# geoeo/ORB_SLAM3_V1.0

Hardware: AMD Instinct MI355X
Metric: frames/sec ORB extract+match, 752x480 8-level 1000-feat; bit-exact kp/desc (higher is better)
Workload: dtype u8

## Files before the change

### orb_slam3_v1.0_amd/csrc/kernels_pyramid.hip

```cpp
#include <algorithm>
#include <cstdlib>

#include "launch.h"

namespace orbfe {

constexpr int kRsTW = 128, kRsTH = 16;
constexpr int kRsMaxRows = 40, kRsMaxCols = 304;

template <int KPASS>
__global__ __launch_bounds__(256) void resize_kernel(const uint8_t* __restrict__ src, size_t srcFrameStride,
                                                     int sw, int sh, int spitch, int srcAligned4,
                                                     uint8_t* __restrict__ dst, size_t dstFrameStride,
                                                     int dw, int dh, int dpitch,
                                                     const uint32_t* __restrict__ xtab,
                                                     const uint32_t* __restrict__ ytab)
{
    __shared__ __attribute__((aligned(16))) uint8_t sSrc[kRsMaxRows][kRsMaxCols];

    const int f = blockIdx.x;
    const int tx0 = blockIdx.y * kRsTW;
    const int ty0 = blockIdx.z * kRsTH;
    const int tid = threadIdx.x;
    const uint8_t* s = src + (size_t)f * srcFrameStride;

    const int x0 = tx0 + (tid & 31) * 4;
    const int yA = ty0 + (tid >> 5), yB = yA + 8;
    const bool colOk = x0 < dw;
    uint4 xt4 = make_uint4(0, 0, 0, 0);
    uint32_t ytA = 0, ytB = 0;
    if (colOk) xt4 = *reinterpret_cast<const uint4*>(xtab + x0);
    if (yA < dh) ytA = ytab[yA];
    if (yB < dh) ytB = ytab[yB];

    const int txLast = min(tx0 + kRsTW, dw) - 1;
    const int tyLast = min(ty0 + kRsTH, dh) - 1;
    const int sx0 = (int)(xtab[tx0] & 0xffffu) & ~3;
    const int sx1 = min((int)(xtab[txLast] & 0xffffu) + 1, sw - 1);
    const int sy0 = (int)(ytab[ty0] & 0xffffu);
    const int sy1 = min((int)(ytab[tyLast] & 0xffffu) + 1, sh - 1);
    const int nrows = sy1 - sy0 + 1;
    const int ndw = (sx1 - sx0) / 4 + 1;
    const bool staged = nrows <= 4 * KPASS && ndw * 4 <= kRsMaxCols;

    if (staged) {
        const int c4l = tid & 63, rl = tid >> 6;
        if (srcAligned4 && ndw <= 64) {
            constexpr int kPass = KPASS;
            const bool cok = c4l < ndw;
            uint32_t off = __umul24((unsigned)(sy0 + rl), (unsigned)spitch) + (unsigned)(sx0 + 4 * c4l);
            const uint32_t step = 4u * (unsigned)spitch;
            uint32_t wv[kPass];
#pragma unroll
            for (int k = 0; k < kPass; k++) {
                wv[k] = 0;
                if (cok && rl + 4 * k < nrows) wv[k] = *reinterpret_cast<const uint32_t*>(s + off);
                off += step;
            }
#pragma unroll
            for (int k = 0; k < kPass; k++)
                if (cok && rl + 4 * k < nrows) *reinterpret_cast<uint32_t*>(&sSrc[rl + 4 * k][4 * c4l]) = wv[k];
        } else {
            for (int r = rl; r < nrows; r += 4) {
                const uint8_t* row = s + (size_t)(sy0 + r) * spitch;
                for (int c4 = c4l; c4 < ndw; c4 += 64) {
                    const int gx = sx0 + 4 * c4;
                    uint32_t wv = 0;
#pragma unroll
                    for (int i = 0; i < 4; i++)
                        if (gx + i < sw) wv |= (uint32_t)row[gx + i] << (8 * i);
                    *reinterpret_cast<uint32_t*>(&sSrc[r][4 * c4]) = wv;
                }
            }
        }
        __syncthreads();
    }
    if (!colOk) return;

    const uint32_t xt[4] = {xt4.x, xt4.y, xt4.z, xt4.w};
    const int nvalid = min(4, dw - x0);
    auto body = [&](auto fetch) {
#pragma unroll
        for (int half = 0; half < 2; half++) {
            const int y = half ? yB : yA;
            if (y >= dh) continue;
            const uint32_t yt = half ? ytB : ytA;
            const int y1 = (int)(yt & 0xffffu);
            const uint32_t wy = yt >> 16;
            const int y2 = min(y1 + 1, sh - 1);
            uint32_t outw = 0;
            const uint32_t wyc = 2048u - wy;
#pragma unroll
            for (int i = 0; i < 4; i++) {
                const int x1 = (int)(xt[i] & 0xffffu);
                const uint32_t wx = xt[i] >> 16;
                const uint32_t wxc = 2048u - wx;
                const int x2 = min(x1 + 1, sw - 1);
                const uint32_t a = fetch(y1, x1), b = fetch(y1, x2), c = fetch(y2, x1), e = fetch(y2, x2);
                const uint32_t top = __umul24(a, wxc) + __umul24(b, wx);
                const uint32_t bot = __umul24(c, wxc) + __umul24(e, wx);
                const uint32_t v = __umul24(top, wyc) + __umul24(bot, wy) + (1u << 21);
                outw |= (v >> 22) << (8 * i);
            }
            uint8_t* d = dst + (size_t)f * dstFrameStride + __umul24((unsigned)y, (unsigned)dpitch);
            if (nvalid == 4) {
                *reinterpret_cast<uint32_t*>(d + x0) = outw;
            } else {
                for (int i = 0; i < nvalid; i++) d[x0 + i] = (uint8_t)(outw >> (8 * i));
            }
        }
    };
    if (staged)
        body([&](int yy, int xx) -> uint32_t {
            return (&sSrc[0][0])[__umul24((uint32_t)(yy - sy0), (uint32_t)kRsMaxCols) + (uint32_t)(xx - sx0)];
        });
    else
        body([&](int yy, int xx) -> uint32_t { return s[(size_t)yy * spitch + xx]; });
}


constexpr int kPyrWaves = 4;

constexpr int kPyrRows = 7;
constexpr int kPyrSegDw = 96;
constexpr int kPyrStride = 128;


__device__ __forceinline__ uint32_t mad24_vsv(uint32_t a, uint32_t w, uint32_t c)
{
    uint32_t r;
    asm("v_mad_u32_u24 %0, %1, %2, %3" : "=v"(r) : "v"(a), "s"(w), "v"(c));
    return r;
}

__device__ __forceinline__ void pyr_hpass(uint32_t d0, uint32_t d1, uint32_t d2, const uint32_t (&sel)[4], const uint32_t (&wp)[4],
                                          uint32_t (&h)[4])
{
    typedef unsigned short us2 __attribute__((ext_vector_type(2)));
    const uint32_t e0 = __builtin_amdgcn_alignbyte(d1, d0, 3), e1 = __builtin_amdgcn_alignbyte(d2, d1, 3);
#pragma unroll
    for (int i = 0; i < 4; i++) {
        const uint32_t pair = i < 3 ? __builtin_amdgcn_perm(d1, d0, sel[i]) : __builtin_amdgcn_perm(e1, e0, sel[i]);
        h[i] = __builtin_amdgcn_udot2(__builtin_bit_cast(us2, pair), __builtin_bit_cast(us2, wp[i]), 0u, false);
    }
}

__global__ __launch_bounds__(kPyrWaves * 64) void pyramid_kernel(const PipelineDesc* __restrict__ P, int l, int R,
                                                                 const uint8_t* __restrict__ gray0, size_t gray0FrameStride,
                                                                 int gray0Pitch, uint8_t* __restrict__ ws,
                                                                 const uint32_t* __restrict__ tabs)
{
    __shared__ uint32_t sRows[kPyrWaves][kPyrRows][kPyrStride];

    const int f = blockIdx.x;
    const int lane = threadIdx.x & 63;
    const int wave = __builtin_amdgcn_readfirstlane((int)(threadIdx.x >> 6));
    uint32_t* const ring = &sRows[wave][0][0];

    {
        const LevelDesc& S = P->lv[l - 1];
        const LevelDesc& D = P->lv[l];
        const int sw = S.w, sh = S.h, dw = D.w, dh = D.h, dpitch = D.pitch;
        const uint8_t* src = l == 1 ? gray0 + (size_t)f * gray0FrameStride : ws + S.imgOff + (size_t)f * S.imgFrameStride;
        const int spitch = l == 1 ? gray0Pitch : S.pitch;
        uint8_t* dst = ws + D.imgOff + (size_t)f * D.imgFrameStride;
        const uint32_t* xtab = tabs + D.xtabOff;
        const uint32_t* ytab = tabs + D.ytabOff;
        const int strips = (dh + R - 1) / R, chunks = (dw + 255) / 256;
        const __amdgpu_buffer_rsrc_t srsrc =
            __builtin_amdgcn_make_buffer_rsrc(const_cast<uint8_t*>(src), 0, (sh - 1) * spitch + ((sw + 3) & ~3), 0x00020000);
        const __amdgpu_buffer_rsrc_t drsrc = __builtin_amdgcn_make_buffer_rsrc(dst, 0, dh * dpitch, 0x00020000);

        const int task = (int)blockIdx.y * kPyrWaves + wave;
        if (task < strips * chunks) {
            const int strip = task / chunks, chunk = task - strip * chunks;
            const int x0 = chunk * 256 + lane * 4;
            const bool colOk = x0 < dw;
            const int xg = min(x0, (dw - 1) & ~3);
            const uint4 xt4 = *reinterpret_cast<const uint4*>(xtab + xg);
            const uint32_t xt[4] = {xt4.x, xt4.y, xt4.z, xt4.w};
            const uint32_t start = (xt[0] & 0xffffu) & ~3u;
            const uint32_t segBase = (xtab[chunk * 256] & 0xffffu) & ~3u;
            const uint32_t winOff = start - segBase;
            uint32_t sel[4], wp[4];
#pragma unroll
            for (int i = 0; i < 4; i++) {
                const uint32_t o = (xt[i] & 0xffffu) - start - (i == 3 ? 3u : 0u);
                sel[i] = 0x0c000c00u | o | ((o + 1u) << 16);
                const uint32_t wx = xt[i] >> 16;
                wp[i] = (2048u - wx) | (wx << 16);
            }
            const int nvalid = min(4, dw - x0);
            constexpr uint32_t kNowhere = 0x7ffffff0u;
            const uint32_t rowEnd = (uint32_t)((sw + 3) & ~3);
            const uint32_t colA = segBase + 4u * (uint32_t)lane;
            const uint32_t ldA = colA + 4u <= rowEnd ? colA : kNowhere;
            const uint32_t ldB = (lane < kPyrSegDw - 64 && colA + 260u <= rowEnd) ? colA + 256u : kNowhere;
            const uint32_t stX = colOk ? (uint32_t)x0 : kNowhere;
            const bool partial = (dw & 3) != 0;

            const int ys = strip * R, ye = min(ys + R, dh);
            const uint32_t roMax = (uint32_t)((sh - 1) * spitch);
            uint32_t kRound = 1u << 23;
            asm("" : "+v"(kRound));
            uint32_t ytN[4];
            uint32_t ga[kPyrRows], gb[kPyrRows];
            auto request = [&](int yb) {
                const uint4 y4 = *reinterpret_cast<const uint4*>(ytab + yb);
                ytN[0] = y4.x; ytN[1] = y4.y; ytN[2] = y4.z; ytN[3] = y4.w;
                uint32_t ro = (ytN[0] & 0xffffu) * (uint32_t)spitch;
#pragma unroll
                for (int j = 0; j < kPyrRows; j++) {
                    const uint32_t roc = min(ro, roMax);
                    ga[j] = __builtin_amdgcn_raw_buffer_load_b32(srsrc, ldA, roc, 0);
                    gb[j] = __builtin_amdgcn_raw_buffer_load_b32(srsrc, ldB, roc, 0);
                    ro += (uint32_t)spitch;
                }
            };
            request(ys);
            uint32_t stRow = (uint32_t)(ys * dpitch);
#pragma unroll 1
            for (int yb = ys; yb < ye; yb += 4) {
                uint32_t yt[4];
#pragma unroll
                for (int k = 0; k < 4; k++) yt[k] = ytN[k];
                const int rA = (int)(yt[0] & 0xffffu);
#pragma unroll
                for (int j = 0; j < kPyrRows; j++) {
                    ring[j * kPyrStride + lane] = ga[j];
                    ring[j * kPyrStride + 64 + lane] = gb[j];
                }
                if (yb + 4 < ye) request(yb + 4);
#pragma unroll
                for (int k = 0; k < 4; k++) {
                    const int jt = (int)(yt[k] & 0xffffu) - rA;
                    const uint32_t* wt = reinterpret_cast<const uint32_t*>(reinterpret_cast<const uint8_t*>(ring + jt * kPyrStride) + winOff);
                    const uint32_t* wb = wt + kPyrStride;
                    uint32_t hT[4], hB[4];
                    pyr_hpass(wt[0], wt[1], wt[2], sel, wp, hT);
                    pyr_hpass(wb[0], wb[1], wb[2], sel, wp, hB);
                    const uint32_t wy4 = (yt[k] >> 16) * 4u, wyc4 = 8192u - wy4;
                    uint32_t v[4];
#pragma unroll
                    for (int i = 0; i < 4; i++) v[i] = mad24_vsv(hB[i], wy4, mad24_vsv(hT[i], wyc4, kRound));
                    const uint32_t lo = __builtin_amdgcn_perm(v[1], v[0], 0x0c0c0703u);
                    const uint32_t hi = __builtin_amdgcn_perm(v[3], v[2], 0x0c0c0703u);
                    const uint32_t outw = lo | (hi << 16);
                    if (yb + k < ye) {
                        if (!partial) {
                            __builtin_amdgcn_raw_buffer_store_b32(outw, drsrc, stX, stRow, 0);
                        } else if (colOk) {
                            if (nvalid == 4) {
                                __builtin_amdgcn_raw_buffer_store_b32(outw, drsrc, (uint32_t)x0, stRow, 0);
                            } else {
                                for (int i = 0; i < nvalid; i++)
                                    __builtin_amdgcn_raw_buffer_store_b8((uint8_t)(outw >> (8 * i)), drsrc, (uint32_t)(x0 + i), stRow, 0);
                            }
                        }
                    }
                    stRow += (uint32_t)dpitch;
                }
            }
        }
    }
}

void launch_resize(hipStream_t s, int frames, const uint8_t* src, size_t srcFrameStride, int sw, int sh,
                   int spitch, int srcAligned4, uint8_t* dst, size_t dstFrameStride, int dw, int dh, int dpitch,
                   const uint32_t* xtab, const uint32_t* ytab)
{
    dim3 block(256);
    dim3 grid(frames, (dw + kRsTW - 1) / kRsTW, (dh + kRsTH - 1) / kRsTH);
    const int maxRows = (int)(((long long)(kRsTH - 1) * sh + dh - 1) / dh) + 2;
    if (maxRows <= 24)
        hipLaunchKernelGGL(resize_kernel<6>, grid, block, 0, s, src, srcFrameStride, sw, sh, spitch, srcAligned4, dst,
                           dstFrameStride, dw, dh, dpitch, xtab, ytab);
    else
        hipLaunchKernelGGL(resize_kernel<kRsMaxRows / 4>, grid, block, 0, s, src, srcFrameStride, sw, sh, spitch, srcAligned4,
                           dst, dstFrameStride, dw, dh, dpitch, xtab, ytab);
}


bool pyramid_level_fits(const uint32_t* xtab, const uint32_t* ytab, int sw, int sh, int dw, int dh)
{
    for (int y = 0; y < dh; y++) {
        if ((int)(ytab[y] & 0xffffu) + 1 > sh - 1) return false;
        const int yl = std::min(y + 3, dh - 1);
        if ((int)(ytab[yl] & 0xffffu) + 1 - (int)(ytab[y] & 0xffffu) + 1 > kPyrRows) return false;
    }
    for (int c0 = 0; c0 < dw; c0 += 256) {
        const uint32_t segBase = (xtab[c0] & 0xffffu) & ~3u;
        const int xl = (std::min(c0 + 256, dw) - 1) & ~3;
        const uint32_t startL = (xtab[xl] & 0xffffu) & ~3u;
        if (startL + 12 - segBase > 4u * kPyrSegDw) return false;
    }
    for (int x0 = 0; x0 < dw; x0 += 4) {
        const uint32_t start = (xtab[x0] & 0xffffu) & ~3u;
        for (int i = 0; i < 4 && x0 + i < dw; i++) {
            const uint32_t x1 = xtab[x0 + i] & 0xffffu;
            if ((int)x1 + 1 > sw - 1 || x1 < start) return false;
            const uint32_t o = x1 - start;
            if (i < 3 ? o + 1 > 7 : (o < 3 || o - 3 + 1 > 7)) return false;
        }
    }
    return true;
}

void launch_pyramid_level(hipStream_t s, int frames, const PipelineDesc* dP, int level, int dw, int dh, const uint8_t* gray0,
                          size_t gray0FrameStride, int gray0Pitch, uint8_t* ws, const uint32_t* tabs)
{
#ifdef ORBFE_DIAG
    static const int envR = getenv("ORBFE_PYR_ROWS") ? atoi(getenv("ORBFE_PYR_ROWS")) : 0;
#else
    constexpr int envR = 0;
#endif
    const int R = envR > 0 ? (envR + 3) & ~3 : frames >= 128 ? 8 : 4;
    const int tasks = ((dh + R - 1) / R) * ((dw + 255) / 256);
    hipLaunchKernelGGL(pyramid_kernel, dim3(frames, (tasks + kPyrWaves - 1) / kPyrWaves), dim3(kPyrWaves * 64), 0, s, dP, level, R, gray0,
                       gray0FrameStride, gray0Pitch, ws, tabs);
}


namespace {

struct ChainCtx {
    const uint8_t* src0;
    int pitch0, w0, h0;
    const uint32_t* xtab[3];
    const uint32_t* ytab[3];
    int w[3], h[3];
};

template <int K>
__device__ __forceinline__ uint32_t chain_px(const ChainCtx& c, int x, int y)
{
    const uint32_t xt = c.xtab[K - 1][x], yt = c.ytab[K - 1][y];
    const int sw = K == 1 ? c.w0 : c.w[K - 2], sh = K == 1 ? c.h0 : c.h[K - 2];
    const int x1 = (int)(xt & 0xffffu), y1 = (int)(yt & 0xffffu);
    const uint32_t wx = xt >> 16, wy = yt >> 16;
    const uint32_t wxc = 2048u - wx, wyc = 2048u - wy;
    const int x2 = min(x1 + 1, sw - 1), y2 = min(y1 + 1, sh - 1);
    uint32_t a, b, cc, e;
    if constexpr (K == 1) {
        const uint8_t* r1 = c.src0 + (size_t)y1 * c.pitch0;
        const uint8_t* r2 = c.src0 + (size_t)y2 * c.pitch0;
        a = r1[x1]; b = r1[x2]; cc = r2[x1]; e = r2[x2];
    } else {
        a = chain_px<K - 1>(c, x1, y1); b = chain_px<K - 1>(c, x2, y1);
        cc = chain_px<K - 1>(c, x1, y2); e = chain_px<K - 1>(c, x2, y2);
    }
    const uint32_t top = __umul24(a, wxc) + __umul24(b, wx);
    const uint32_t bot = __umul24(cc, wxc) + __umul24(e, wx);
    const uint32_t v = __umul24(top, wyc) + __umul24(bot, wy) + (1u << 21);
    return v >> 22;
}

__global__ __launch_bounds__(256) void pyramid_chain_kernel(const PipelineDesc* __restrict__ P, int l0, int depth,
                                                            const uint8_t* __restrict__ gray0, size_t gray0FrameStride, int gray0Pitch,
                                                            uint8_t* __restrict__ ws, const uint32_t* __restrict__ tabs,
                                                            uint32_t* __restrict__ zero, int nZeroPerFrame)
{
    const int f = blockIdx.y;
    if (zero && blockIdx.x == 0)
        for (int i = threadIdx.x; i < nZeroPerFrame; i += 256) zero[(size_t)f * nZeroPerFrame + i] = 0;
    ChainCtx c;
    const LevelDesc& S = P->lv[l0];
    c.src0 = l0 == 0 ? gray0 + (size_t)f * gray0FrameStride : ws + S.imgOff + (size_t)f * S.imgFrameStride;
    c.pitch0 = l0 == 0 ? gray0Pitch : S.pitch;
    c.w0 = S.w;
    c.h0 = S.h;
    int np[3] = {0, 0, 0};
#pragma unroll
    for (int k = 0; k < 3; k++) {
        const LevelDesc& D = P->lv[min(l0 + 1 + k, P->nLevels - 1)];
        c.xtab[k] = tabs + D.xtabOff;
        c.ytab[k] = tabs + D.ytabOff;
        c.w[k] = D.w;
        c.h[k] = D.h;
        np[k] = k < depth ? D.w * D.h : 0;
    }
    int idx = (int)blockIdx.x * 256 + (int)threadIdx.x;
    int k = 0;
    if (idx >= np[0]) { idx -= np[0]; k = 1; if (idx >= np[1]) { idx -= np[1]; k = 2; if (idx >= np[2]) return; } }
    const LevelDesc& D = P->lv[l0 + 1 + k];
    const int y = idx / D.w, x = idx - y * D.w;
    uint32_t out;
    if (k == 0) out = chain_px<1>(c, x, y);
    else if (k == 1) out = chain_px<2>(c, x, y);
    else out = chain_px<3>(c, x, y);
    ws[D.imgOff + (size_t)f * D.imgFrameStride + (size_t)y * D.pitch + x] = (uint8_t)out;
}

}

void launch_pyramid_chain(hipStream_t s, int frames, const PipelineDesc* dP, const PipelineDesc& hostP, int l0, int depth,
                          const uint8_t* gray0, size_t gray0FrameStride, int gray0Pitch, uint8_t* ws, const uint32_t* tabs,
                          uint32_t* zero, int nZeroPerFrame)
{
    long long pixels = 0;
    for (int k = 0; k < depth; k++) {
        const LevelDesc& D = hostP.lv[l0 + 1 + k];
        pixels += (long long)D.w * D.h;
    }
    hipLaunchKernelGGL(pyramid_chain_kernel, dim3((unsigned)((pixels + 255) / 256), frames), dim3(256), 0, s, dP, l0, depth, gray0,
                       gray0FrameStride, gray0Pitch, ws, tabs, zero, nZeroPerFrame);
}

}
```

Baseline: 226,900.

## Stream pyramid rows through a two-slot LDS ring and reuse horizontal passes across rows

The pyramid kernel stops staging all seven source rows per quad into a 7-row LDS ring. Each row is now written into a double-buffered two-row slot, horizontally filtered once, and the result is carried forward as hPrev. Output rows are emitted as soon as their bottom row's pass is ready, and a row already filtered by the previous quad is skipped via the carry check. It also prefetches the ytab quads ahead, interleaves the next quad's global loads with the per-row work, and simplifies tail stores. This cuts LDS footprint and duplicate horizontal filtering, but adds a stricter monotonic-ytab fit check and more complex control flow.

```diff
diff --git a/orb_slam3_v1.0_amd/csrc/kernels_pyramid.hip b/orb_slam3_v1.0_amd/csrc/kernels_pyramid.hip
--- a/orb_slam3_v1.0_amd/csrc/kernels_pyramid.hip
+++ b/orb_slam3_v1.0_amd/csrc/kernels_pyramid.hip
@@ -1,5 +1,6 @@
 #include <algorithm>
 #include <cstdlib>
+#include <type_traits>
 
 #include "launch.h"
 
@@ -123,7 +124,8 @@
 
 constexpr int kPyrRows = 7;
 constexpr int kPyrSegDw = 96;
-constexpr int kPyrStride = 128;
+constexpr int kPyrSlack = kPyrRows - 5;
+constexpr int kPyrMinLast = 4;
 
 
 __device__ __forceinline__ uint32_t mad24_vsv(uint32_t a, uint32_t w, uint32_t c)
@@ -150,7 +152,7 @@
                                                                  int gray0Pitch, uint8_t* __restrict__ ws,
                                                                  const uint32_t* __restrict__ tabs)
 {
-    __shared__ uint32_t sRows[kPyrWaves][kPyrRows][kPyrStride];
+    __shared__ uint32_t sRows[kPyrWaves][2][kPyrSegDw];
 
     const int f = blockIdx.x;
     const int lane = threadIdx.x & 63;
@@ -190,25 +192,34 @@
                 const uint32_t wx = xt[i] >> 16;
                 wp[i] = (2048u - wx) | (wx << 16);
             }
-            const int nvalid = min(4, dw - x0);
             constexpr uint32_t kNowhere = 0x7ffffff0u;
             const uint32_t rowEnd = (uint32_t)((sw + 3) & ~3);
             const uint32_t colA = segBase + 4u * (uint32_t)lane;
             const uint32_t ldA = colA + 4u <= rowEnd ? colA : kNowhere;
             const uint32_t ldB = (lane < kPyrSegDw - 64 && colA + 260u <= rowEnd) ? colA + 256u : kNowhere;
-            const uint32_t stX = colOk ? (uint32_t)x0 : kNowhere;
-            const bool partial = (dw & 3) != 0;
+            const uint32_t stX = x0 + 4 <= dw ? (uint32_t)x0 : kNowhere;
+            const uint32_t stT = (colOk && x0 + 4 > dw) ? (uint32_t)x0 : kNowhere;
+            const int tailN = dw & 3;
+            const bool tail = tailN != 0 && chunk == chunks - 1;
+            uint32_t* const wrA = ring + lane;
+            uint32_t* const wrB = ring + (lane < kPyrSegDw - 64 ? 64 + lane : lane);
+            const uint32_t* const rdW = reinterpret_cast<const uint32_t*>(reinterpret_cast<const uint8_t*>(ring) + winOff);
 
             const int ys = strip * R, ye = min(ys + R, dh);
+            const int yQuadLast = (dh - 1) & ~3;
             const uint32_t roMax = (uint32_t)((sh - 1) * spitch);
             uint32_t kRound = 1u << 23;
             asm("" : "+v"(kRound));
-            uint32_t ytN[4];
+            uint32_t yt[4], ytN[4];
+            {
+                const uint4 q0 = *reinterpret_cast<const uint4*>(ytab + ys);
+                const uint4 q1 = *reinterpret_cast<const uint4*>(ytab + min(ys + 4, yQuadLast));
+                yt[0] = q0.x; yt[1] = q0.y; yt[2] = q0.z; yt[3] = q0.w;
+                ytN[0] = q1.x; ytN[1] = q1.y; ytN[2] = q1.z; ytN[3] = q1.w;
+            }
             uint32_t ga[kPyrRows], gb[kPyrRows];
-            auto request = [&](int yb) {
-                const uint4 y4 = *reinterpret_cast<const uint4*>(ytab + yb);
-                ytN[0] = y4.x; ytN[1] = y4.y; ytN[2] = y4.z; ytN[3] = y4.w;
-                uint32_t ro = (ytN[0] & 0xffffu) * (uint32_t)spitch;
+            {
+                uint32_t ro = (yt[0] & 0xffffu) * (uint32_t)spitch;
 #pragma unroll
                 for (int j = 0; j < kPyrRows; j++) {
                     const uint32_t roc = min(ro, roMax);
@@ -216,29 +227,25 @@
                     gb[j] = __builtin_amdgcn_raw_buffer_load_b32(srsrc, ldB, roc, 0);
                     ro += (uint32_t)spitch;
                 }
-            };
-            request(ys);
+            }
+            asm volatile("" : "+v"(ga[0]), "+v"(gb[0]), "+v"(ga[1]), "+v"(gb[1]), "+v"(ga[2]), "+v"(gb[2]), "+v"(ga[3]), "+v"(gb[3]),
+                              "+v"(ga[4]), "+v"(gb[4]), "+v"(ga[5]), "+v"(gb[5]), "+v"(ga[6]), "+v"(gb[6]));
+            static_assert(kPyrRows == 7, "the operand list above names every staged row");
+            uint32_t hPrev[4] = {0u, 0u, 0u, 0u};
+            int passed = -1;
             uint32_t stRow = (uint32_t)(ys * dpitch);
-#pragma unroll 1
-            for (int yb = ys; yb < ye; yb += 4) {
-                uint32_t yt[4];
-#pragma unroll
-                for (int k = 0; k < 4; k++) yt[k] = ytN[k];
+            auto step = [&](const int yb, auto moreTag) {
+                constexpr bool more = decltype(moreTag)::value;
+                uint4 q2 = make_uint4(0, 0, 0, 0);
+                if (more) q2 = *reinterpret_cast<const uint4*>(ytab + min(yb + 8, yQuadLast));
                 const int rA = (int)(yt[0] & 0xffffu);
-#pragma unroll
-                for (int j = 0; j < kPyrRows; j++) {
-                    ring[j * kPyrStride + lane] = ga[j];
-                    ring[j * kPyrStride + 64 + lane] = gb[j];
-                }
-                if (yb + 4 < ye) request(yb + 4);
-#pragma unroll
-                for (int k = 0; k < 4; k++) {
-                    const int jt = (int)(yt[k] & 0xffffu) - rA;
-                    const uint32_t* wt = reinterpret_cast<const uint32_t*>(reinterpret_cast<const uint8_t*>(ring + jt * kPyrStride) + winOff);
-                    const uint32_t* wb = wt + kPyrStride;
-                    uint32_t hT[4], hB[4];
-                    pyr_hpass(wt[0], wt[1], wt[2], sel, wp, hT);
-                    pyr_hpass(wb[0], wb[1], wb[2], sel, wp, hB);
+                int jt[4];
+#pragma unroll
+                for (int k = 0; k < 4; k++) jt[k] = (int)(yt[k] & 0xffffu) - rA;
+                const int jLast = jt[3] + 1;
+                const bool carry = rA == passed;
+                uint32_t roN = (ytN[0] & 0xffffu) * (uint32_t)spitch;
+                auto emit = [&](int k, const uint32_t (&hT)[4], const uint32_t (&hB)[4]) {
                     const uint32_t wy4 = (yt[k] >> 16) * 4u, wyc4 = 8192u - wy4;
                     uint32_t v[4];
 #pragma unroll
@@ -246,21 +253,48 @@
                     const uint32_t lo = __builtin_amdgcn_perm(v[1], v[0], 0x0c0c0703u);
                     const uint32_t hi = __builtin_amdgcn_perm(v[3], v[2], 0x0c0c0703u);
                     const uint32_t outw = lo | (hi << 16);
-                    if (yb + k < ye) {
-                        if (!partial) {
-                            __builtin_amdgcn_raw_buffer_store_b32(outw, drsrc, stX, stRow, 0);
-                        } else if (colOk) {
-                            if (nvalid == 4) {
-                                __builtin_amdgcn_raw_buffer_store_b32(outw, drsrc, (uint32_t)x0, stRow, 0);
-                            } else {
-                                for (int i = 0; i < nvalid; i++)
-                                    __builtin_amdgcn_raw_buffer_store_b8((uint8_t)(outw >> (8 * i)), drsrc, (uint32_t)(x0 + i), stRow, 0);
-                            }
-                        }
+                    const uint32_t so = stRow + (uint32_t)(k * dpitch);
+                    __builtin_amdgcn_raw_buffer_store_b32(outw, drsrc, stX, so, 0);
+                    if (tail) {
+                        __builtin_amdgcn_raw_buffer_store_b8((uint8_t)outw, drsrc, stT, so, 0);
+                        if (tailN > 1) __builtin_amdgcn_raw_buffer_store_b8((uint8_t)(outw >> 8), drsrc, stT, so + 1u, 0);
+                        if (tailN > 2) __builtin_amdgcn_raw_buffer_store_b8((uint8_t)(outw >> 16), drsrc, stT, so + 2u, 0);
                     }
-                    stRow += (uint32_t)dpitch;
+                };
+#pragma unroll
+                for (int j = 0; j < kPyrRows; j++) {
+                    if (j == 0 ? !carry : (j <= kPyrMinLast || j <= jLast)) {
+                        const int bo = (j & 1) * kPyrSegDw;
+                        wrB[bo] = gb[j];
+                        wrA[bo] = ga[j];
+                        uint32_t hCur[4];
+                        pyr_hpass(rdW[bo], rdW[bo + 1], rdW[bo + 2], sel, wp, hCur);
+#pragma unroll
+                        for (int k = 0; k < 4; k++)
+                            if (j >= k + 1 && j <= k + 1 + kPyrSlack)
+                                if (jt[k] + 1 == j && (more || yb + k < ye)) emit(k, hPrev, hCur);
+#pragma unroll
+                        for (int i = 0; i < 4; i++) hPrev[i] = hCur[i];
+                    }
+                    if (more) {
+                        const uint32_t roc = min(roN, roMax);
+                        ga[j] = __builtin_amdgcn_raw_buffer_load_b32(srsrc, ldA, roc, 0);
+                        gb[j] = __builtin_amdgcn_raw_buffer_load_b32(srsrc, ldB, roc, 0);
+                        roN += (uint32_t)spitch;
+                    }
                 }
-            }
+                if (more) {
+                    passed = rA + max(jLast, kPyrMinLast);
+                    stRow += 4u * (uint32_t)dpitch;
+#pragma unroll
+                    for (int k = 0; k < 4; k++) yt[k] = ytN[k];
+                    ytN[0] = q2.x; ytN[1] = q2.y; ytN[2] = q2.z; ytN[3] = q2.w;
+                }
+            };
+            int yb = ys;
+#pragma unroll 1
+            for (; yb + 4 < ye; yb += 4) step(yb, std::true_type());
+            step(yb, std::false_type());
         }
     }
 }
@@ -284,9 +318,11 @@
 bool pyramid_level_fits(const uint32_t* xtab, const uint32_t* ytab, int sw, int sh, int dw, int dh)
 {
     for (int y = 0; y < dh; y++) {
-        if ((int)(ytab[y] & 0xffffu) + 1 > sh - 1) return false;
-        const int yl = std::min(y + 3, dh - 1);
-        if ((int)(ytab[yl] & 0xffffu) + 1 - (int)(ytab[y] & 0xffffu) + 1 > kPyrRows) return false;
+        const int y1 = (int)(ytab[y] & 0xffffu);
+        if (y1 + 1 > sh - 1) return false;
+        if (y + 1 < dh && (int)(ytab[y + 1] & 0xffffu) < y1) return false;
+        const int k = y & 3, jt = y1 - (int)(ytab[y - k] & 0xffffu);
+        if (jt < k || jt > k + kPyrSlack) return false;
     }
     for (int c0 = 0; c0 < dw; c0 += 256) {
         const uint32_t segBase = (xtab[c0] & 0xffffu) & ~3u;
```

New measurement: 229,200 (median of 3 runs). No clear change (+1.0%).
